# foollh/PicoPose

Measured on AMD Instinct MI355X. Metric: image-crops/sec (224x224, 162 templates), higher is better.
Workload: dtype f32 tensors; networks: f32 operands split into 2 f16 terms (22 bits) on f16 MFMA with f32 accumulate; stage-1 contraction: f16 MFMA operands, f32 accumulate, exact f32 re-evaluation of near-ties; PnP f64

## Files before the change

### include/picopose_hip.h

```cpp
#ifndef PICOPOSE_HIP_H
#define PICOPOSE_HIP_H

#include <stddef.h>
#include <stdint.h>

#ifdef __cplusplus
extern "C" {
#endif

#define PP_OK 0
#define PP_EINVAL (-1)
#define PP_EWORKSPACE (-2)
#define PP_ELAUNCH (-3)

#define PP_MATCH_EXACT 0
#define PP_MATCH_FAST 1

const char* pp_strerror(int code);
int pp_version(void);

int pp_prof_enable(int max_records);
int pp_prof_collect(float* out_ms, int max_out, int* count);
int pp_prof_gemm_enable(int max_records);
int pp_prof_gemm_collect(double* ms, double* flops, int* launches);
// ... 16 lines not shown
int pp_stage1_scores_ex(const void* bank, int bank_dtype, const float* query, const float* mask,
                        int mask_h, int mask_w, int B, int N, int C, int mode,
                        float eps, void* workspace, size_t workspace_bytes,
                        float* sim_avg, int32_t* stats, void* stream);

int pp_topk(const float* scores, int B, int N, int k, float* out_score,
            int64_t* out_index, void* stream);

int pp_stage1_match(const float* bank, const float* query, const float* mask,
                    int mask_h, int mask_w, int B, int N, int C, int k, int mode,
                    float eps, void* workspace, size_t workspace_bytes,
                    float* sim_avg, float* out_score, int64_t* out_index,
                    int32_t* stats, void* stream);
int pp_stage1_match_ex(const void* bank, int bank_dtype, const float* query, const float* mask,
                       int mask_h, int mask_w, int B, int N, int C, int k, int mode,
                       float eps, void* workspace, size_t workspace_bytes, float* sim_avg,
                       float* out_score, int64_t* out_index, int32_t* stats, void* stream);

int pp_stage1_indexed_workspace_bytes(int B, int N, int C, size_t* bytes);
int pp_stage1_scores_indexed(const void* bank, int bank_dtype, const int64_t* obj_index, int n_obj,
                             const float* query, const float* mask, int mask_h, int mask_w, int B, int N,
                             int C, int mode, float eps, void* workspace, size_t workspace_bytes,
                             float* sim_avg, int32_t* stats, void* stream);
int pp_stage1_match_indexed(const void* bank, int bank_dtype, const int64_t* obj_index, int n_obj,
                            const float* query, const float* mask, int mask_h, int mask_w, int B, int N,
                            int C, int k, int mode, float eps, void* workspace, size_t workspace_bytes,
                            float* sim_avg, float* out_score, int64_t* out_index, int32_t* stats,
                            void* stream);



int pp_similarity_volume(const float* src_feat, const float* tar_feat, const float* src_mask,
                         int mask_h, int mask_w, int B, int C, float* out, void* stream);

int pp_calc_pred_Ms(const float* pred_scale, const float* pred_inplane, const float* pred_translation,
                    const float* tem_pose, const float* tem_K, const float* tem_M, int B,
                    float trans_scale, float* pred_Ms, void* stream);

int pp_pose_recovery_2d(const float* query_M, const float* query_K, const float* pred_Ms,
                        const float* tem_K, const float* tem_M, const float* tem_pose, int B,
                        float* pred_pose, void* stream);

int pp_init_correspondences(const float* pred_Ms, const float* tem_mask, int mask_h, int mask_w, int B,
                            float* init_flow, float* init_certainty, void* stream);

int pp_stage3_correspondences(const float* pred_flow, const float* pred_certainty, int B, int H, int W,
                              float threshold, int64_t* tar_pts, int64_t* src_pts, void* stream);

int pp_gather_valid(const float* features, const int64_t* index_patches, int B, int C, int H, int W,
                    int N, float* out, int32_t* count, void* stream);

#define PP_ACT_NONE 0
#define PP_ACT_RELU 1
#define PP_ACT_GELU 2
#define PP_ACT_LEAKY01 3
#define PP_ACT_TANH 4

#define PP_PREC_F32 0
#define PP_PREC_F16X3 1
#define PP_PREC_F16 2

typedef struct PpGemmDesc {
    const float* A;
    const float* B;
    float* C;
    const float* bias;
// ... 46 lines not shown
int pp_split_weights_t(const float* w, long long n, int terms, void* out, float* scale, void* stream);
int pp_split_activation_t(const float* x, long long batch_stride, int B, int P, int row_stride, int C, int relu, void* out,
                          int ld_h, int terms, void* stream);
int pp_hl_patch_columns_t(const float* x, int ld_x, int c, long long rows, void* out, int ld_h, int col0, int terms, void* stream);
int pp_layernorm_t(const float* x, const float* gamma, const float* beta, int rows, int C, float eps, float* y, void* out, int terms,
                   void* stream);
int pp_resize_bilinear_nhwc_t(const float* in, int B, int H, int W, int C, int Ho, int Wo, float mul, void* out, int terms,
                              void* stream);
int pp_resize_bilinear_nhwc_dual(const float* in, int B, int H, int W, int C, int Ho, int Wo, float mul, float* out, void* out_operand,
                                 int terms, void* stream);
int pp_warp_nhwc_t(const float* feat, int feat_batch, const float* flow, int B, int H, int W, int C, int ld_flow, void* out,
                   int ld_h, int terms, void* stream);
int pp_attention_t(const void* qkv_operand, int terms, int B, int T, int heads, int head_dim, float scale, float* out,
                   void* out_operand, void* stream);

int pp_attention(const float* qkv, int B, int T, int heads, int head_dim, float scale, float* out, void* stream);
int pp_attention_split(const float* qkv, int B, int T, int heads, int head_dim, float scale, float* out, void* out_hl,
                       void* stream);
int pp_attention_ex(const float* qkv, int B, int T, int heads, int head_dim, float scale, int prec, float* out, void* out_hl,
                    void* stream);
int pp_attention_hl(const void* qkv_hl, int B, int T, int heads, int head_dim, float scale, float* out, void* out_hl,
                    void* stream);
int pp_attention_train(const float* qkv, int B, int T, int heads, int head_dim, float scale, float* out, float* lse2, void* stream);
int pp_attention_backward(const float* qkv, const float* out, const float* dout, const float* lse2, const float* gpair, int B, int T,
                          int heads, int head_dim, float scale, float* Dws, float* dqkv, void* stream);

int pp_layernorm(const float* x, const float* gamma, const float* beta, int rows, int C, float eps,
                 float* y, void* stream);
int pp_layernorm_split(const float* x, const float* gamma, const float* beta, int rows, int C, float eps, float* y,
                       void* hl, void* stream);
int pp_softmax_rows(float* x, int rows, int n, int ld, void* stream);
int pp_groupnorm_nhwc(const float* x, const float* gamma, const float* beta, int B, int HW, int C,
                      int groups, float eps, int relu, float* y, void* stream);
int pp_transpose_batched(const float* in, long long in_batch_stride, int B, int R, int C, float* out,
                         long long out_batch_stride, int ld_out, int col_off, void* stream);
int pp_assemble_tokens(const float* patches, const float* cls_token, const float* pos, int B, int T, int C,
                       float* tokens, void* stream);
int pp_normalize_rows(const float* x, int rows, int n, float eps, float* y, void* stream);

int pp_resize_bilinear_nhwc(const float* in, int B, int H, int W, int C, int Ho, int Wo, float mul,
                            float* out, void* stream);
int pp_resize_bilinear_nhwc_hl(const float* in, int B, int H, int W, int C, int Ho, int Wo, float mul, void* out_hl,
                               void* stream);
int pp_warp_nhwc(const float* feat, int feat_batch, const float* flow, int B, int H, int W, int C, int ld_flow,
                 float* out, int ld_out, void* stream);
int pp_warp_nhwc_hl(const float* feat, int feat_batch, const float* flow, int B, int H, int W, int C, int ld_flow,
                    void* out_hl, int ld_h, void* stream);
int pp_avgpool2_nhwc(const float* in, int B, int H, int W, int C, float* out, void* stream);
int pp_gather_rows(const float* src, const long long* index, long long n_src_rows, long long row_floats, int n, float* dst,
                   void* stream);
int pp_bank_rows_to_tokens(const float* bank, long long n_bank_rows, int C, int P, const long long* index, int n, float* tokens, int ld,
                           int T, int skip, void* stream);
int pp_patch_operand(const float* bank, long long n_bank_rows, const long long* index, int n, const float* front, int n_front, int H, int W,
                     void* out, int terms, void* stream);
int pp_flow_operand(const float* flow, int ld_flow, long long rows, void* out8, int terms, void* stream);

int pp_crop_resize_normalize(const unsigned char* image, int H, int W, const unsigned char* mask, int y1, int y2, int x1,
                             int x2, int S, int rgb_mask_flag, const double* mean3, const double* std3, float* out_rgb,
                             float* out_mask, void* stream);
int pp_depth_points_nearest(const float* depth_m, int H, int W, int y1, int y2, int x1, int x2, int P, float fx, float fy,
                            float cx, float cy, float* out_pts, void* stream);
int pp_corr_lookup_nhwc(const float* f1, int ld_f1, const float* f2_l0, const float* f2_l1, const float* f2_l2,
                        int f2_batch, const float* flow, int B, int H, int W, int C, int levels, int radius,
                        int ld_flow, float* out, int ld_out, void* stream);
int pp_corr_lookup_nhwc_ex(const float* f1, int ld_f1, const float* f2_l0, const float* f2_l1, const float* f2_l2,
                           int f2_batch, const float* flow, int B, int H, int W, int C, int levels, int radius,
// ... 322 lines not shown
```

### picopose_amd/csrc/pp_gemm.hip

```cpp

#include <hip/hip_runtime.h>
#include <stdint.h>
#include <stdio.h>
#include <stdlib.h>
#include <atomic>
#include <mutex>
#include <string>
#include <unordered_map>
#include "../../include/picopose_hip.h"
#include "pp_common.h"
#include "pp_reduce_dev.h"
#include "pp_gemm_dev.h"
#include "pp_gemm_u.h"

static std::mutex g_tune_mu;
static std::unordered_map<std::string, int> g_tune_best;
static int g_tune_loaded = 0;

static int tune_load_locked(const char* path) {
    FILE* f = fopen(path, "r");
    if (!f) return -1;
    char key[192];
    int cfg, n = 0;
    while (fscanf(f, "%191s %d", key, &cfg) == 2) {
// ... 607 lines not shown
static void launch_layernorm(const float* x, const float* gamma, const float* beta, int rows, int C, float eps, float* y,
                             _Float16* hl, hipStream_t st, int terms = 2) {
    const dim3 grid((rows + 3) / 4), block(256);
    const bool vec = C % 8 == 0 && ((uintptr_t)x % 16 == 0) && ((uintptr_t)gamma % 16 == 0) &&
                     ((uintptr_t)beta % 16 == 0) && (!y || (uintptr_t)y % 16 == 0) && (!hl || (uintptr_t)hl % 16 == 0);
    if (vec && C <= 512)
        hipLaunchKernelGGL(layernorm_kernel<1>, grid, block, 0, st, x, gamma, beta, rows, C, eps, y, hl, terms);
    else if (vec && C <= 1024)
        hipLaunchKernelGGL(layernorm_kernel<2>, grid, block, 0, st, x, gamma, beta, rows, C, eps, y, hl, terms);
    else
        hipLaunchKernelGGL(layernorm_kernel<0>, grid, block, 0, st, x, gamma, beta, rows, C, eps, y, hl, terms);
}

__global__ __launch_bounds__(256) void softmax_kernel(float* __restrict__ x, int rows, int n, int ld) {
    const int row = blockIdx.x * 4 + (threadIdx.x >> 6), lane = threadIdx.x & 63;
    if (row >= rows) return;
    float* xr = x + (size_t)row * ld;
    float mx = -INFINITY;
    for (int c = lane; c < n; c += 64) mx = fmaxf(mx, xr[c]);
    mx = wave_max(mx);
    float s = 0.f;
    for (int c = lane; c < n; c += 64) {
        const float e = expf(xr[c] - mx);
        xr[c] = e;
        s += e;
    }
    s = wave_sum(s);
    const float inv = 1.0f / s;
    for (int c = lane; c < n; c += 64) xr[c] *= inv;
}

__global__ __launch_bounds__(256) void groupnorm_kernel(const float* __restrict__ x, const float* __restrict__ g,
                                                        const float* __restrict__ b, int HW, int C, int G, float eps,
                                                        int relu, float* __restrict__ y) {
    __shared__ float red[8];
    const int img = blockIdx.x / G, grp = blockIdx.x % G, cg = C / G, tid = threadIdx.x;
    const float* xi = x + (size_t)img * HW * C + grp * cg;
    float* yi = y + (size_t)img * HW * C + grp * cg;
    const int n = HW * cg;
    float s = 0.f;
    for (int i = tid; i < n; i += 256) s += xi[(size_t)(i / cg) * C + (i % cg)];
    const float mean = block_reduce_all<4>(s, red, op_sum{}) / (float)n;
    float v = 0.f;
    for (int i = tid; i < n; i += 256) {
        const float dlt = xi[(size_t)(i / cg) * C + (i % cg)] - mean;
        v = fmaf(dlt, dlt, v);
    }
    const float rstd = 1.0f / sqrtf(block_reduce_all<4>(v, red + 4, op_sum{}) / (float)n + eps);
    for (int i = tid; i < n; i += 256) {
        const int c = i % cg;
        const size_t off = (size_t)(i / cg) * C + c;
        float o = (xi[off] - mean) * rstd * g[grp * cg + c] + b[grp * cg + c];
        if (relu) o = o > 0.f ? o : 0.f;
        yi[off] = o;
    }
}

__global__ __launch_bounds__(256) void transpose_kernel(const float* __restrict__ in, long long in_bs, int R,
                                                        int Cc, float* __restrict__ out, long long out_bs,
                                                        int ld_out, int col_off) {
    __shared__ float t[32][33];
    const int b = blockIdx.z, r0 = blockIdx.y * 32, c0 = blockIdx.x * 32;
    const int tx = threadIdx.x & 31, ty = threadIdx.x >> 5;
    const float* ib = in + (size_t)b * in_bs;
    float* ob = out + (size_t)b * out_bs;
#pragma unroll
    for (int i = 0; i < 4; ++i) {
        const int r = r0 + ty + 8 * i, c = c0 + tx;
        if (r < R && c < Cc) t[ty + 8 * i][tx] = ib[(size_t)r * Cc + c];
    }
    __syncthreads();
#pragma unroll
    for (int i = 0; i < 4; ++i) {
        const int c = c0 + ty + 8 * i, r = r0 + tx;
        if (r < R && c < Cc) ob[(size_t)c * ld_out + col_off + r] = t[tx][ty + 8 * i];
    }
}

__global__ __launch_bounds__(256) void assemble_tokens_kernel(const float* __restrict__ patches,
                                                              const float* __restrict__ cls,
                                                              const float* __restrict__ pos, int T, int C,
                                                              float* __restrict__ tokens) {
    const int t = blockIdx.x, b = blockIdx.y;
    const float* src = t == 0 ? cls : patches + ((size_t)b * T + (t - 1)) * C;
    float* dst = tokens + ((size_t)b * (T + 1) + t) * C;
    for (int c = threadIdx.x; c < C; c += 256) dst[c] = src[c] + pos[(size_t)t * C + c];
}
// ... 638 lines not shown
    return (int)g_tune_best.size();
}

int pp_layernorm(const float* x, const float* gamma, const float* beta, int rows, int C, float eps, float* y,
                 void* stream) {
    if (!x || !gamma || !beta || !y || rows <= 0 || C <= 0) return PP_EINVAL;
    launch_layernorm(x, gamma, beta, rows, C, eps, y, nullptr, (hipStream_t)stream);
    return pp_last_launch();
}

int pp_layernorm_t(const float* x, const float* gamma, const float* beta, int rows, int C, float eps, float* y,
                   void* hl, int terms, void* stream) {
    if (!x || !gamma || !beta || !hl || rows <= 0 || C <= 0 || C % 8 != 0 || (terms != 1 && terms != 2)) return PP_EINVAL;
    launch_layernorm(x, gamma, beta, rows, C, eps, y, (_Float16*)hl, (hipStream_t)stream, terms);
    return pp_last_launch();
}

int pp_layernorm_split(const float* x, const float* gamma, const float* beta, int rows, int C, float eps, float* y,
                       void* hl, void* stream) {
    return pp_layernorm_t(x, gamma, beta, rows, C, eps, y, hl, 2, stream);
}

int pp_softmax_rows(float* x, int rows, int n, int ld, void* stream) {
    if (!x || rows <= 0 || n <= 0 || ld < n) return PP_EINVAL;
    hipLaunchKernelGGL(softmax_kernel, dim3((rows + 3) / 4), dim3(256), 0, (hipStream_t)stream, x, rows, n, ld);
    return pp_last_launch();
}

int pp_groupnorm_nhwc(const float* x, const float* gamma, const float* beta, int B, int HW, int C, int groups,
                      float eps, int relu, float* y, void* stream) {
    if (!x || !gamma || !beta || !y || B <= 0 || HW <= 0 || C <= 0 || groups <= 0 || C % groups != 0)
        return PP_EINVAL;
    hipLaunchKernelGGL(groupnorm_kernel, dim3(B * groups), dim3(256), 0, (hipStream_t)stream, x, gamma, beta, HW,
                       C, groups, eps, relu, y);
    return pp_last_launch();
}

int pp_transpose_batched(const float* in, long long in_batch_stride, int B, int R, int C, float* out,
                         long long out_batch_stride, int ld_out, int col_off, void* stream) {
    if (!in || !out || B <= 0 || R <= 0 || C <= 0 || ld_out < R + col_off || col_off < 0) return PP_EINVAL;
    if (in_batch_stride == 0) in_batch_stride = (long long)R * C;
    if (out_batch_stride == 0) out_batch_stride = (long long)C * ld_out;
    hipLaunchKernelGGL(transpose_kernel, dim3((C + 31) / 32, (R + 31) / 32, B), dim3(256), 0,
                       (hipStream_t)stream, in, in_batch_stride, R, C, out, out_batch_stride, ld_out, col_off);
    return pp_last_launch();
}

int pp_assemble_tokens(const float* patches, const float* cls_token, const float* pos, int B, int T, int C,
                       float* tokens, void* stream) {
    if (!patches || !cls_token || !pos || !tokens || B <= 0 || T <= 0 || C <= 0) return PP_EINVAL;
    hipLaunchKernelGGL(assemble_tokens_kernel, dim3(T + 1, B), dim3(256), 0, (hipStream_t)stream, patches,
                       cls_token, pos, T, C, tokens);
    return pp_last_launch();
}

int pp_normalize_rows(const float* x, int rows, int n, float eps, float* y, void* stream) {
    if (!x || !y || rows <= 0 || n <= 0 || n > 64) return PP_EINVAL;
    hipLaunchKernelGGL(normalize_rows_kernel, dim3((rows + 255) / 256), dim3(256), 0, (hipStream_t)stream, x,
                       rows, n, eps, y);
    return pp_last_launch();
}

}
```

### picopose_amd/csrc/pp_geom.hip

```cpp

#include <hip/hip_runtime.h>
#include <stdint.h>
#include "../../include/picopose_hip.h"
#include "pp_common.h"

namespace {

typedef float f32x16 __attribute__((ext_vector_type(16)));
typedef float f4 __attribute__((ext_vector_type(4)));

__device__ __forceinline__ int nearest16(int dst, int in) {
    int i = (int)floorf((float)dst * ((float)in / 16.0f));
    return i < in - 1 ? i : in - 1;
}

__global__ __launch_bounds__(256) void simvol_kernel(const float* __restrict__ src,
                                                     const float* __restrict__ tar,
                                                     const float* __restrict__ src_mask, int mh,
                                                     int mw, int C, float* __restrict__ out) {
    __shared__ __attribute__((aligned(16))) float Qs[16 * 128];
    __shared__ __attribute__((aligned(16))) float Xs[16 * 128];
    __shared__ float rq[128], rx[128];
    const int b = blockIdx.x, t0 = blockIdx.y * 128, s0 = blockIdx.z * 128;
    const int tid = threadIdx.x, lane = tid & 63, w = tid >> 6;
    const int wr = w >> 1, wc = w & 1, l31 = lane & 31, lh = lane >> 5;
    const float* qg = tar + (size_t)b * C * 256 + t0;
    const float* xg = src + (size_t)b * C * 256 + s0;
    f32x16 acc[2][2];
#pragma unroll
    for (int i = 0; i < 2; ++i)
#pragma unroll
        for (int j = 0; j < 2; ++j)
#pragma unroll
            for (int r = 0; r < 16; ++r) acc[i][j][r] = 0.f;
    float sa[2] = {0.f, 0.f}, sb[2] = {0.f, 0.f};
    for (int c0 = 0; c0 < C; c0 += 16) {
#pragma unroll
        for (int j = 0; j < 2; ++j) {
            const int idx = tid + 256 * j, row = idx >> 5, col = (idx & 31) * 4;
            *(f4*)(Qs + row * 128 + col) = *(const f4*)(qg + (size_t)(c0 + row) * 256 + col);
            *(f4*)(Xs + row * 128 + col) = *(const f4*)(xg + (size_t)(c0 + row) * 256 + col);
        }
        __syncthreads();
#pragma unroll
        for (int p = 0; p < 8; ++p) {
            float a[2], bv[2];
#pragma unroll
            for (int i = 0; i < 2; ++i) {
                a[i] = Qs[(2 * p + lh) * 128 + wr * 64 + i * 32 + l31];
                bv[i] = Xs[(2 * p + lh) * 128 + wc * 64 + i * 32 + l31];
                sa[i] = fmaf(a[i], a[i], sa[i]);
                sb[i] = fmaf(bv[i], bv[i], sb[i]);
            }
#pragma unroll
            for (int i = 0; i < 2; ++i)
#pragma unroll
                for (int j = 0; j < 2; ++j)
                    acc[i][j] = __builtin_amdgcn_mfma_f32_32x32x2f32(a[i], bv[j], acc[i][j], 0, 0, 0);
        }
        __syncthreads();
    }
#pragma unroll
    for (int i = 0; i < 2; ++i) {
        sa[i] += __shfl_xor(sa[i], 32);
        sb[i] += __shfl_xor(sb[i], 32);
    }
    if (lh == 0) {
        if (wc == 0) {
            rq[wr * 64 + l31] = 1.0f / fmaxf(sqrtf(sa[0]), 1e-12f);
            rq[wr * 64 + 32 + l31] = 1.0f / fmaxf(sqrtf(sa[1]), 1e-12f);
        }
        if (wr == 0) {
#pragma unroll
            for (int i = 0; i < 2; ++i) {
                const int s = s0 + wc * 64 + i * 32 + l31;
                const float m = src_mask[((size_t)b * mh + nearest16(s >> 4, mh)) * mw + nearest16(s & 15, mw)];
                rx[wc * 64 + i * 32 + l31] = m / fmaxf(sqrtf(sb[i]), 1e-12f);
            }
        }
    }
    __syncthreads();
#pragma unroll
    for (int j = 0; j < 2; ++j) {
        const int sl = wc * 64 + j * 32 + l31;
        const float cs = rx[sl];
        float* o = out + ((size_t)b * 256 + s0 + sl) * 256;
#pragma unroll
        for (int i = 0; i < 2; ++i)
#pragma unroll
            for (int e = 0; e < 16; ++e) {
                const int tl = wr * 64 + i * 32 + (e & 3) + 8 * (e >> 2) + 4 * lh;
                const int t = t0 + tl;
                float v = acc[i][j][e] * rq[tl] * cs;
                v = v < 0.f ? 0.f : v;
                o[(t & 15) * 16 + (t >> 4)] = v;
            }
    }
}

struct M3 {
    float m[9];
};
__device__ __forceinline__ M3 ld3(const float* p) {
    M3 r;
#pragma unroll
    for (int i = 0; i < 9; ++i) r.m[i] = p[i];
    return r;
}
__device__ __forceinline__ M3 mul3(const M3& a, const M3& b) {
    M3 r;
#pragma unroll
    for (int i = 0; i < 3; ++i)
#pragma unroll
        for (int j = 0; j < 3; ++j)
            r.m[i * 3 + j] = a.m[i * 3] * b.m[j] + a.m[i * 3 + 1] * b.m[3 + j] + a.m[i * 3 + 2] * b.m[6 + j];
    return r;
}
__device__ __forceinline__ void mulv3(const M3& a, const float* v, float* o) {
#pragma unroll
    for (int i = 0; i < 3; ++i) o[i] = a.m[i * 3] * v[0] + a.m[i * 3 + 1] * v[1] + a.m[i * 3 + 2] * v[2];
}

__global__ void pred_ms_kernel(const float* __restrict__ scale, const float* __restrict__ inplane,
                               const float* __restrict__ trans, const float* __restrict__ tem_pose,
                               const float* __restrict__ tem_K, const float* __restrict__ tem_M, int B,
                               float trans_scale, float* __restrict__ out) {
    const int b = blockIdx.x * blockDim.x + threadIdx.x;
    if (b >= B) return;
    const float* P = tem_pose + (size_t)b * 16;
    const float t[3] = {P[3], P[7], P[11]};
// ... 117 lines not shown
            y = ib[2 * n + 1];
        }
        const bool v = x != -1 && y != -1;
        const unsigned long long bal = __ballot(v);
        const int pre = __popcll(bal & ((1ull << lane) - 1ull));
        if (lane == 0) wsum[wv] = __popcll(bal);
        __syncthreads();
        int off = base;
        for (int i = 0; i < wv; ++i) off += wsum[i];
        if (v) {
            const int r = off + pre;
            const int64_t p = y * W + x;
            for (int c = 0; c < C; ++c) ob[(size_t)r * C + c] = fb[(size_t)c * H * W + p];
        }
        __syncthreads();
        if (tid == 0) {
            int t = base;
            for (int i = 0; i < 16; ++i) t += wsum[i];
            base = t;
        }
        __syncthreads();
    }
    if (tid == 0) count[b] = base;
}

}

extern "C" {

int pp_similarity_volume(const float* src_feat, const float* tar_feat, const float* src_mask, int mask_h,
                         int mask_w, int B, int C, float* out, void* stream) {
    if (!src_feat || !tar_feat || !src_mask || !out) return PP_EINVAL;
    if (B <= 0 || C <= 0 || C % 16 != 0 || mask_h <= 0 || mask_w <= 0) return PP_EINVAL;
    hipLaunchKernelGGL(simvol_kernel, dim3(B, 2, 2), dim3(256), 0, (hipStream_t)stream, src_feat, tar_feat,
                       src_mask, mask_h, mask_w, C, out);
    return pp_last_launch();
}

int pp_calc_pred_Ms(const float* pred_scale, const float* pred_inplane, const float* pred_translation,
                    const float* tem_pose, const float* tem_K, const float* tem_M, int B, float trans_scale,
                    float* pred_Ms, void* stream) {
    if (!pred_scale || !pred_inplane || !pred_translation || !tem_pose || !tem_K || !tem_M || !pred_Ms || B <= 0)
        return PP_EINVAL;
    hipLaunchKernelGGL(pred_ms_kernel, dim3((B + 63) / 64), dim3(64), 0, (hipStream_t)stream, pred_scale,
                       pred_inplane, pred_translation, tem_pose, tem_K, tem_M, B, trans_scale, pred_Ms);
    return pp_last_launch();
}

int pp_pose_recovery_2d(const float* query_M, const float* query_K, const float* pred_Ms, const float* tem_K,
                        const float* tem_M, const float* tem_pose, int B, float* pred_pose, void* stream) {
    if (!query_M || !query_K || !pred_Ms || !tem_K || !tem_M || !tem_pose || !pred_pose || B <= 0)
        return PP_EINVAL;
    hipLaunchKernelGGL(pose2d_kernel, dim3((B + 63) / 64), dim3(64), 0, (hipStream_t)stream, query_M, query_K,
                       pred_Ms, tem_K, tem_M, tem_pose, B, pred_pose);
    return pp_last_launch();
}

int pp_init_correspondences(const float* pred_Ms, const float* tem_mask, int mask_h, int mask_w, int B,
                            float* init_flow, float* init_certainty, void* stream) {
    if (!pred_Ms || !tem_mask || !init_flow || !init_certainty || B <= 0) return PP_EINVAL;
    if (mask_h != mask_w || mask_h < 16) return PP_EINVAL;
    hipLaunchKernelGGL(init_corr_kernel, dim3(B), dim3(256), 0, (hipStream_t)stream, pred_Ms, tem_mask,
                       mask_h, mask_w, init_flow, init_certainty);
    return pp_last_launch();
}

int pp_stage3_correspondences(const float* pred_flow, const float* pred_certainty, int B, int H, int W,
                              float threshold, int64_t* tar_pts, int64_t* src_pts, void* stream) {
// ... 17 lines not shown
```

### picopose_amd/model/stage2.py

```python
import torch

from .. import ops
from .common import Packed, conv_p, linear_p, norm_p, seq


def _head(hidden, out):
    return seq((0, linear_p(hidden, hidden)), (2, linear_p(hidden, hidden)), (4, linear_p(hidden, out)))


class AffineRegressor(Packed):
    def __init__(self, cfg, use_tanh_act=True, normalize_output=True):
        super().__init__()
        self.in_channel, self.hidden_dim = cfg.in_channel, cfg.hidden_dim
        self.feat_size = 8
        hd = self.hidden_dim
        self.features = seq((0, conv_p(self.in_channel, hd, 1)), (1, norm_p(hd)), (3, conv_p(hd, hd, 3, bias=False)),
                            (4, norm_p(hd)))
        self.fc1 = linear_p(hd * self.feat_size * self.feat_size, 1024)
        self.fc2 = linear_p(1024, 256)
        self.translation_predictor = _head(hd, 2)
        self.scale_predictor = _head(hd, 1)
        self.inplane_predictor = _head(hd, 2)

    def _pack(self):
        f = self.features
        hd, fs = self.hidden_dim, self.feat_size
        fc1 = self.fc1.weight.float().view(-1, hd, fs, fs).permute(0, 2, 3, 1).reshape(-1, fs * fs * hd).contiguous()
        return {"c0": ops.pack_conv_weight(getattr(f, "0").weight.float()),
                "c3": ops.pack_conv_weight(getattr(f, "3").weight.float()), "fc1": fc1}

    def _mlp(self, head, x, last_act=None):
        l0, l2, l4 = getattr(head, "0"), getattr(head, "2"), getattr(head, "4")
        x = ops.linear(x, l0.weight, l0.bias, act="relu")
        x = ops.linear(x, l2.weight, l2.bias, act="relu")
        return ops.linear(x, l4.weight, l4.bias, act=last_act)

    def forward(self, x):
        with torch.no_grad():
            pk, f = self.packed(), self.features
            B = x.shape[0]
            h = ops.conv2d(ops.to_nhwc(x), pk["c0"], getattr(f, "0").bias, 1)
            h = ops.groupnorm(h, getattr(f, "1").weight, getattr(f, "1").bias, 32, relu=True)
            h = ops.conv2d(h, pk["c3"], None, 3, stride=2, pad=1)
            h = ops.groupnorm(h, getattr(f, "4").weight, getattr(f, "4").bias, 32, relu=True)
            h = ops.linear_splitk(h.view(B, -1), pk["fc1"], self.fc1.bias, act="leaky01")
            h = ops.linear(h, self.fc2.weight, self.fc2.bias, act="leaky01")
            translation = self._mlp(self.translation_predictor, h)
            scale = self._mlp(self.scale_predictor, h)
            inplane = ops.normalize_rows(self._mlp(self.inplane_predictor, h, last_act="tanh"))
            return translation, scale.squeeze(1), inplane
```

### picopose_amd/ops.py

```python
import contextlib
import ctypes
import os
import threading

import torch

from . import _lib
from ._lib import PpGemmDesc

ACT = {None: 0, "none": 0, "relu": 1, "gelu": 2, "leaky01": 3, "tanh": 4}

PRECISION = "f16x3"
_PREC = {"f32": 0, "f16x3": 1, "f16": 2}
_split_cache = {}
_scope = threading.local()


def precision():
    return getattr(_scope, "mode", None) or PRECISION


def check_precision(mode):
    if mode is not None and mode not in _PREC:
        raise ValueError(f"unknown arithmetic mode {mode!r}: expected None or one of {sorted(_PREC)}")
# ... 892 lines not shown
        out = torch.empty(B * T, heads * hd, dtype=torch.float32, device=dev)
    if isinstance(qkv, Split):
        _lib.call("pp_attention_t", qkv.hl, qkv.terms, B, T, heads, hd, float(hd) ** -0.5, out, sp.hl if sp else None)
    else:
        assert qkv.is_contiguous()
        if sp is not None and sp.terms == 1:
            sp, out = None, torch.empty(B * T, heads * hd, dtype=torch.float32, device=dev)
        _lib.call("pp_attention_ex", qkv, B, T, heads, hd, float(hd) ** -0.5, _fly_prec(), out, sp.hl if sp else None)
    if sp is not None:
        _chk(sp.hl, "pp_attention")
    return sp if sp is not None else out


def layernorm(x, weight, bias, eps, out_split=False):
    rows, C = x.shape
    assert x.is_contiguous()
    if out_split and _split_ok(C):
        sp = Split.empty(rows, C, x.device)
        _lib.call("pp_layernorm_t", x, weight, bias, rows, C, float(eps), None, sp.hl, sp.terms)
        _chk(sp.hl, "pp_layernorm_t")
        return sp
    y = torch.empty_like(x)
    _lib.call("pp_layernorm", x, weight, bias, rows, C, float(eps), y)
    return y


def softmax_rows_(x):
    assert x.is_contiguous()
    n = x.shape[-1]
    _lib.call("pp_softmax_rows", x, x.numel() // n, n, n)
    return x


def groupnorm(x, weight, bias, groups, eps=1e-5, relu=False):
    B, H, W, C = x.shape
    assert x.is_contiguous()
    y = torch.empty_like(x)
    _lib.call("pp_groupnorm_nhwc", x, weight, bias, B, H * W, C, groups, float(eps), int(relu), y)
    return y


def batchnorm_train(x, bn, relu=False, residual=None, residual2=None, eps=1e-5, momentum=0.1):
    assert x.is_contiguous() and x.dtype == torch.float32
    C = x.shape[-1]
    rows = x.numel() // C
    nbytes = _lib.lib().pp_batchnorm_train_workspace_bytes(rows, C)
    ws = torch.empty(nbytes, dtype=torch.uint8, device=x.device)
    y = torch.empty_like(x)
    for r in (residual, residual2):
        assert r is None or (r.is_contiguous() and r.shape == x.shape)
    _lib.call("pp_batchnorm_train", x, bn.weight, bn.bias, rows, C, float(eps), float(momentum), bn.running_mean, bn.running_var,
              int(relu), residual, residual2, y, ws, nbytes)
    bn.num_batches_tracked += 1
    return y


def to_nhwc(x, c_pad=None):
    B, C, H, W = x.shape
    x = x.contiguous().float()
    Cp = c_pad if c_pad and c_pad > C else C
    out = (torch.zeros if Cp > C else torch.empty)(B, H, W, Cp, dtype=torch.float32, device=x.device)
    _lib.call("pp_transpose_batched", x, 0, B, C, H * W, out, 0, Cp, 0)
    return out


def to_nchw(x):
    B, H, W, C = x.shape
    assert x.is_contiguous()
    out = torch.empty(B, C, H, W, dtype=torch.float32, device=x.device)
# ... 37 lines not shown
            _chk(tgt.cols(col0, C), "pp_warp_nhwc_t")
        return None
    if out is None:
        out = torch.empty(B, H, W, C, dtype=torch.float32, device=feat.device)
    _lib.call("pp_warp_nhwc", feat, Bf, flow, B, H, W, C, flow.stride(2), out, out.stride(2))
    return out


def avgpool2(x):
    B, H, W, C = x.shape
    assert x.is_contiguous()
    out = torch.empty(B, H // 2, W // 2, C, dtype=torch.float32, device=x.device)
    _lib.call("pp_avgpool2_nhwc", x, B, H, W, C, out)
    return out


def avgpool2_hl(x, keep_f32=True):
    B, H, W, C = x.shape
    assert x.is_contiguous() and C % 8 == 0 and terms() == 2
    out = torch.empty(B, H // 2, W // 2, C, dtype=torch.float32, device=x.device) if keep_f32 else None
    sp = Split.empty(B * (H // 2) * (W // 2), C, x.device)
    sp.image = (B, H // 2, W // 2)
    _lib.call("pp_avgpool2_hl", x, B, H, W, C, out, sp.hl)
    _chk(sp.hl, "pp_avgpool2_hl")
    return out, sp


def corr_operand_out():
    return os.environ.get("PP_CORR_OPERAND_OUT", "1") != "0"


def decoder_lean():
    return os.environ.get("PP_DECODER_LEAN", "1") != "0"


def corr_takes_operands(f1_hl, f2_hl, H, W, C):
    return (f1_hl is not None and f2_hl is not None and precision() == "f16x3" and f2_hl.terms == 2 and H % 8 == 0 and W % 8 == 0 and C % 32 == 0
            and os.environ.get("PP_CORR_TILED", "1") != "0" and os.environ.get("PP_CORR_HL", "1") != "0")


def _corr_pyramid(f2, hl0, levels, fused):
    C = f2.shape[3]
    pyr, hls = [f2], [hl0]
    for i in range(levels - 1):
        if fused:
            p, sp = avgpool2_hl(pyr[-1], keep_f32=i < levels - 2)
            hls.append(sp.hl)
        else:
            p = avgpool2(pyr[-1])
            if hl0 is not None:
                hls.append(split_activation(p, p.shape[0], p.shape[1] * p.shape[2], C, p.shape[1] * p.shape[2] * C, C))
        pyr.append(p)
    return pyr + [None, None], hls + [None, None]


def corr_lookup(f1, f2, flow, levels, radius, c_pad=None, f1_hl=None, f2_hl=None, out_split=False):
    (H, W, C), B = f2.shape[1:], flow.shape[0]
    assert f2.is_contiguous() and flow.stride(3) == 1 and B % f2.shape[0] == 0 and tuple(flow.shape[1:3]) == (H, W)
    operands = corr_takes_operands(f1_hl, f2_hl, H, W, C)
    if f1 is None:
        assert operands, "corr_lookup without the fp32 map f1 needs the operand form of both maps (corr_takes_operands)"
    else:
        assert tuple(f1.shape) == (B, H, W, C) and f1.stride(3) == 1 and f1.stride(1) == W * f1.stride(2) and f1.stride(0) == H * f1.stride(1)
    n = levels * (2 * radius + 1) ** 2
    np_ = c_pad if c_pad and c_pad > n else n
    assert not out_split or (operands and np_ % 8 == 0), "corr_lookup(out_split=True) needs the operand branch and a padded channel count"
# ... 77 lines not shown
```

### picopose_amd/picopose.py

```python
import os

import torch
import torch.nn as nn

from . import ops
from .model.stage1 import FeatureExtractor
from .model.stage2 import AffineRegressor
from .model.stage3 import OffsetRegressor
from .utils.augment import aug_gtM_noise
from .utils.correspondence import compute_init_correspondences, compute_stage3_correspondences
from .utils.keypoints import KeypointInput, KeyPointSampler
from .utils.loss_utils import compute_stage_two_loss, flow_level_losses, infonce_rows
from .utils.matching import matching_features_similarity, matching_templates, matching_templates_indexed
from .utils.pose_recovery import pose_recovery_2d_prediction
from .utils.torch_utils import calc_pred_Ms


BATCH_VIT_TRAIN = os.environ.get("PP_BATCH_VIT_TRAIN", "1") != "0"
BATCH_DPT = os.environ.get("PP_BATCH_DPT", "1") != "0"
PREFETCH_QUERY = os.environ.get("PP_PREFETCH_QUERY", "1") != "0"
TEMPLATE_LAST_FROM_BANK = {"0": False, "1": True}.get(os.environ.get("PP_TEMPLATE_LAST_FROM_BANK"))


def _tensor_key(t, fe=None):
    key = (t.data_ptr(), tuple(t.shape), t._version, ops.precision())
    return key if fe is None else key + (fe._signatures()[0],)


def _image_rows(p, b0, b1):
    if isinstance(p, ops.Split):
        hw = p.image[1] * p.image[2]
        s = ops.Split(p.hl[b0 * hw:b1 * hw], p.terms)
        s.image = (b1 - b0,) + tuple(p.image[1:])
        return s
    q = p[b0:b1]
    hl = getattr(p, "_hl", None)
    if hl is not None:
        hw = p.shape[1] * p.shape[2]
        s = ops.Split(hl.hl[b0 * hw:b1 * hw], hl.terms)
        s.image = (b1 - b0, p.shape[1], p.shape[2])
        q._hl = s
    return q


class Net(nn.Module):
    def __init__(self, cfg):
# ... 69 lines not shown
        real_dpt = real[2] if len(real) > 2 else None
        levels = real[3] if len(real) > 3 else None
        output = {"tem_pose": end_points["tem_pose"]}
        output["tar_pts_2d"] = end_points["real_pts2d"].permute(0, 3, 2, 1)
        output["src_pts_3d"] = end_points["tem_pts3d"].permute(0, 3, 1, 2)
        pre = real[4] if len(real) > 4 else None
        bank = end_points.get("tem_bank") if tem_cached is None else None
        T = h0 * w0 + 1
        rgb_rows = end_points.get("tem_rgb_rows")

        def tem_images(front=None):
            if rgb_rows is not None and ops.patch_operand_ok(rgb_rows[0], front):
                return ops.patch_operand(*rgb_rows, front=front)
            tem = end_points["tem_rgb"] if rgb_rows is None else ops.gather_rows(*rgb_rows)
            return tem if front is None else torch.cat([front, tem])

        if tem_cached is None and pre is not None and levels is not None:
            alloc, nxt = pre
            Bn = nxt.shape[0]
            both, _ = fe.forward_tokens(tem_images(nxt), level_out=(alloc, 0), full_depth=None if bank is None else Bn)
            tem_tok = [t[Bn:] for t in both]
            if bank is not None:
                nT = tem_tok[0].shape[0]
                tem_tok[-1] = ops.bank_rows_to_tokens(*bank, T, out=alloc[-1][Bn * T:(Bn + nT) * T]).view(nT, T, -1)
            self._query_stash = (_tensor_key(nxt, fe), [a[:Bn * T].clone() for a in alloc], (h0, w0), nxt)
        elif tem_cached is None:
            tem_tok, _ = fe.forward_tokens(tem_images(), level_out=None if levels is None else (levels, 0),
                                           full_depth=None if bank is None else 0)
            if bank is not None:
                nT = tem_tok[0].shape[0]
                tem_tok[-1] = ops.bank_rows_to_tokens(*bank, T, out=None if levels is None else levels[-1][:nT * T]).view(nT, T, -1)
        else:
            tem_last, tem_dpt = tem_cached
        if tem_cached is None:
            tem_last = ops.tokens_to_nchw(tem_tok[-1], 1, h0, w0) if bank is None else ops.gather_rows(*bank)
        sim = matching_features_similarity(tem_last, ops.tokens_to_nchw(real_tok[-1], 1, h0, w0),
                                           end_points["tem_mask"], end_points["real_mask"])
        pred_translation, pred_scale, pred_inplane = self.affine_regressor(sim)
        pred_Ms = calc_pred_Ms(pred_scale, pred_inplane, pred_translation, end_points["tem_pose"], end_points["tem_K"],
                               end_points["tem_M"])
        output["pred_poses"] = pose_recovery_2d_prediction(end_points["real_M"], end_points["real_K"], pred_Ms,
                                                           end_points["tem_K"], end_points["tem_M"], end_points["tem_pose"])
        init_flow, init_certainty = compute_init_correspondences(pred_Ms, end_points["tem_mask"])
        as_img = lambda t: t[:, 1:].unflatten(1, (h0, w0))
        orr = self.offset_regressor
        if levels is not None and real_dpt is None and tem_cached is None:
            nT, nR = tem_tok[0].shape[0], levels[0].shape[0] // T - tem_tok[0].shape[0]
            both = orr.dpt_head.forward_nhwc([as_img(lv.view(-1, T, lv.shape[1])) for lv in levels], finest_operand_only=True)
            tem_dpt, real_dpt = [_image_rows(p_, 0, nT) for p_ in both], [_image_rows(p_, nT, nT + nR) for p_ in both]
        else:
            if real_dpt is None:
                real_dpt = orr.dpt_head.forward_nhwc([as_img(t) for t in real_tok])
            if tem_cached is None:
                tem_dpt = orr.dpt_head.forward_nhwc([as_img(t) for t in tem_tok])
        flows, certs = orr.flow_decoder.forward_nhwc(tem_dpt, real_dpt, ops.to_nhwc(init_flow), ops.to_nhwc(init_certainty))
        if self.keep_stage3:
            self.last_stage3 = (flows[-1], certs[-1])
        output["pred_tar_pts"], output["pred_src_pts"] = compute_stage3_correspondences(
            ops.to_nchw(flows[-1]), ops.to_nchw(certs[-1]), threshold=0.5)
        return output

    def forward_hypotheses(self, end_points, pred_id_src, real):
        hyp = pred_id_src.shape[1]
        cache = end_points.get("template_cache")
        tidx = end_points.get("template_index")

        def cached(rows, idx):
            if cache is None:
                return None
            obj = (cache["obj_index"] if tidx is None else tidx)[rows]
            return end_points["template_feature"][rows if tidx is None else obj, idx], [m[obj, idx] for m in cache["dpt"]]

        if not self.batch_hypotheses:
            rows = torch.arange(pred_id_src.shape[0], device=pred_id_src.device)
            return [self.forward_test_hyp(self.select_template_data(end_points, pred_id_src, k), real,
                                          cached(rows, pred_id_src[:, k])) for k in range(hyp)]
        real_tok, hw = real[0], real[1]
        real_dpt = real[2] if len(real) > 2 and real[2] is not None else None
        levels = real[3] if len(real) > 3 else None
        B = pred_id_src.shape[0]
        idx = pred_id_src.t().reshape(-1)
        rows = torch.arange(B, device=idx.device).repeat(hyp)
        rep = lambda t: t.repeat(hyp, *([1] * (t.dim() - 1)))
        N = end_points["tem_pose"].shape[1]
        trow = rows if tidx is None else tidx[rows]
        flat = trow * N + idx
        rgb_rows = None
        if (ops.patch_operand_on() and not self.training and cache is None and levels is not None and end_points["tem_rgb"].dim() == 5
                and end_points["tem_rgb"].is_contiguous() and flat.dtype == torch.int64 and ops.patch_operand_ok(end_points["tem_rgb"].flatten(0, 1))):
            rgb_rows = (end_points["tem_rgb"].flatten(0, 1), flat)
        sel = {key: (ops.gather_rows(end_points[key].flatten(0, 1), flat) if end_points[key].is_contiguous()
                     else end_points[key][trow, idx])
               for key in ("tem_pose", "tem_K", "tem_M", "tem_mask", "tem_rgb", "tem_pts3d") if not (key == "tem_rgb" and rgb_rows is not None)}
        if rgb_rows is not None:
            sel["tem_rgb_rows"] = rgb_rows
        if self._last_from_bank(end_points):
            sel["tem_bank"] = (end_points["template_feature"].flatten(0, 1), flat)
        for key in ("real_pts2d", "real_K", "real_M", "real_mask", "real_pose"):
            sel[key] = rep(end_points[key])
        toks = ([rep(t) for t in real_tok] if real_dpt is None and levels is None
                else [None] * (len(real_tok) - 1) + [rep(real_tok[-1])])
        out = self.forward_test_hyp(sel, (toks, hw, real_dpt, levels if cache is None else None, real[4] if len(real) > 4 and cache is None else None),
                                    cached(rows, idx))
        return [{key: v[k * B:(k + 1) * B] for key, v in out.items()} for k in range(hyp)]

    TEMPLATE_KEYS = ("template_feature", "tem_pose", "tem_K", "tem_M", "tem_mask", "tem_rgb", "tem_pts3d")

    def _check_template_index(self, end_points):
        tidx = end_points["template_index"]
        B = end_points["real_rgb"].shape[0]
        if not isinstance(tidx, torch.Tensor) or tidx.dtype != torch.int64 or tuple(tidx.shape) != (B,) or tidx.device != end_points["real_rgb"].device:
            raise ValueError(f"template_index must be a ({B},) int64 tensor on the crops' device")
        lead = {key: tuple(end_points[key].shape[:2]) for key in self.TEMPLATE_KEYS if key in end_points}
        if len(set(lead.values())) != 1:
            raise ValueError(f"with template_index every template tensor is (O, N, ...) for the same O and N: {lead}")
        cache = end_points.get("template_cache")
        if cache is not None and cache["obj_index"] is not tidx and not torch.equal(cache["obj_index"].to(tidx.device), tidx):
            raise ValueError("template_cache['obj_index'] and template_index name different objects")

    def forward_test(self, end_points, hyp=5, next_real_rgb=None):
        with torch.no_grad():
            if "template_index" in end_points:
                self._check_template_index(end_points)
            fe = self.feature_extractor
            levels = None
            ops.saturation_word(end_points["real_rgb"].device)
            stash, self._query_stash = getattr(self, "_query_stash", None), None
            if BATCH_DPT and self.batch_hypotheses and end_points.get("template_cache") is None:
                B, _, H, W = end_points["real_rgb"].shape
                T = (H // fe.patch_size) * (W // fe.patch_size) + 1
                pre_ok = PREFETCH_QUERY and next_real_rgb is not None and tuple(next_real_rgb.shape[1:]) == (3, H, W) and next_real_rgb.is_contiguous()
                Bn = next_real_rgb.shape[0] if pre_ok else 0
                alloc = [torch.empty((Bn + (hyp + 1) * B) * T, fe.num_features, dtype=torch.float32, device=end_points["real_rgb"].device)
                         for _ in fe.blocks_to_take]
# ... 97 lines not shown
```

### picopose_amd/utils/matching.py

```python
import torch

from .. import _lib

DEFAULT_MODE = "fast"
_MODES = {"exact": _lib.PP_MATCH_EXACT, "fast": _lib.PP_MATCH_FAST}

_ws_cache = {}


def _workspace(B, N, C, device, query="pp_stage1_workspace_bytes"):
    need = _lib.workspace_bytes(query, B, N, C)
    key = (device.index, torch.cuda.current_stream().cuda_stream)
    ws = _ws_cache.get(key)
    if ws is None or ws.numel() < need:
        ws = torch.empty(need, dtype=torch.uint8, device=device)
        _ws_cache[key] = ws
    return ws, need


def _check_inputs(src_feats, tar_feat, tar_mask):
    if not (src_feats.is_cuda and tar_feat.is_cuda and tar_mask.is_cuda):
        raise _lib.PicoPoseHipError("picopose_amd runs on the GPU only: inputs must be CUDA(HIP) tensors")
    B, N, C, H, W = src_feats.shape
    assert H == W
# ... 101 lines not shown
class MatchingGraph:

    def __init__(self, src_feats, tar_feat, tar_mask, topk=5, mode=None):
        _check_inputs(src_feats, tar_feat, tar_mask)
        for t in (src_feats, tar_feat, tar_mask):
            if not t.is_contiguous():
                raise _lib.PicoPoseHipError("MatchingGraph reads its inputs in place: they must be contiguous")
        if src_feats.dtype not in (torch.float16, torch.float32) or tar_feat.dtype != torch.float32 or tar_mask.dtype != torch.float32:
            raise _lib.PicoPoseHipError("MatchingGraph reads its inputs in place: fp32 query / mask, fp32 or fp16 bank")
        self.inputs = (src_feats, tar_feat, tar_mask)
        self.graph = torch.cuda.CUDAGraph()
        side = torch.cuda.Stream()
        side.wait_stream(torch.cuda.current_stream())
        with torch.cuda.stream(side):
            matching_templates(src_feats, tar_feat, None, tar_mask, topk=topk, mode=mode)
        torch.cuda.current_stream().wait_stream(side)
        with torch.cuda.graph(self.graph):
            self.score, self.index = matching_templates(src_feats, tar_feat, None, tar_mask, topk=topk, mode=mode)

    def __call__(self):
        self.graph.replay()
        return self.score, self.index


def matching_features_similarity(src_feat, tar_feat, src_mask, tar_mask):
    B, C, H, W = src_feat.shape
    assert H == W
    if H != 16:
        raise _lib.PicoPoseHipError("the HIP similarity-volume kernel is built for 16x16 patch grids")
    src, tar, mask = _lib.dev_f32(src_feat, tar_feat, src_mask)
    out = torch.empty(B, H * W, H, W, dtype=torch.float32, device=src.device)
    _lib.call("pp_similarity_volume", src, tar, mask, mask.shape[1], mask.shape[2], B, C, out)
    return out
```

Baseline: 593.4.

## Emit stage-2 similarity volume and groupnorm outputs directly as split f16 operands

The similarity-volume kernel gains an operand mode. It reads query tokens and bank rows in place through an index and writes split f16 GEMM operands directly, which removes the gather_rows, tokens_to_nchw, repeat and later split conversions. The kernel also prefetches the next channel tile into registers so loads overlap compute. Groupnorm and the fc2/MLP first layers emit split outputs as well, which avoids separate conversion passes. The cost is more code paths plus a transposed shared-memory store for the query tile, and the new paths depend on the env flags and presplit mode.

Result: no change. 597.1, median of 6 (+0.6%).

```diff
diff --git a/include/picopose_hip.h b/include/picopose_hip.h
--- a/include/picopose_hip.h
+++ b/include/picopose_hip.h
@@ -72,6 +72,9 @@
 
 int pp_similarity_volume(const float* src_feat, const float* tar_feat, const float* src_mask,
                          int mask_h, int mask_w, int B, int C, float* out, void* stream);
+int pp_similarity_volume_operand(const float* bank, long long n_bank_rows, const long long* index, const float* query_tokens,
+                                 long long query_image_stride, int query_ld, int Bq, const float* src_mask, int mask_h, int mask_w, int B,
+                                 int C, void* out, int terms, void* stream);
 
 int pp_calc_pred_Ms(const float* pred_scale, const float* pred_inplane, const float* pred_translation,
                     const float* tem_pose, const float* tem_K, const float* tem_M, int B,
@@ -184,6 +187,8 @@
 int pp_softmax_rows(float* x, int rows, int n, int ld, void* stream);
 int pp_groupnorm_nhwc(const float* x, const float* gamma, const float* beta, int B, int HW, int C,
                       int groups, float eps, int relu, float* y, void* stream);
+int pp_groupnorm_nhwc_t(const float* x, const float* gamma, const float* beta, int B, int HW, int C, int groups, float eps, int relu,
+                        float* y, void* hl, int terms, void* stream);
 int pp_transpose_batched(const float* in, long long in_batch_stride, int B, int R, int C, float* out,
                          long long out_batch_stride, int ld_out, int col_off, void* stream);
 int pp_assemble_tokens(const float* patches, const float* cls_token, const float* pos, int B, int T, int C,
diff --git a/picopose_amd/csrc/pp_gemm.hip b/picopose_amd/csrc/pp_gemm.hip
--- a/picopose_amd/csrc/pp_gemm.hip
+++ b/picopose_amd/csrc/pp_gemm.hip
@@ -663,7 +663,7 @@
 
 __global__ __launch_bounds__(256) void groupnorm_kernel(const float* __restrict__ x, const float* __restrict__ g,
                                                         const float* __restrict__ b, int HW, int C, int G, float eps,
-                                                        int relu, float* __restrict__ y) {
+                                                        int relu, float* __restrict__ y, _Float16* __restrict__ hl, int terms) {
     __shared__ float red[8];
     const int img = blockIdx.x / G, grp = blockIdx.x % G, cg = C / G, tid = threadIdx.x;
     const float* xi = x + (size_t)img * HW * C + grp * cg;
@@ -683,7 +683,19 @@
         const size_t off = (size_t)(i / cg) * C + c;
         float o = (xi[off] - mean) * rstd * g[grp * cg + c] + b[grp * cg + c];
         if (relu) o = o > 0.f ? o : 0.f;
-        yi[off] = o;
+        if (y) yi[off] = o;
+        if (hl) {
+            _Float16 h, l;
+            pp_split_f16_chk(o, h, l);
+            const size_t row = (size_t)img * HW + i / cg;
+            if (terms == 2) {
+                _Float16* hp = hl + row * 2 * C + pp_hl_col(grp * cg + c, 0);
+                hp[0] = h;
+                hp[8] = l;
+            } else {
+                hl[row * C + grp * cg + c] = h;
+            }
+        }
     }
 }
 
@@ -1388,7 +1400,17 @@
     if (!x || !gamma || !beta || !y || B <= 0 || HW <= 0 || C <= 0 || groups <= 0 || C % groups != 0)
         return PP_EINVAL;
     hipLaunchKernelGGL(groupnorm_kernel, dim3(B * groups), dim3(256), 0, (hipStream_t)stream, x, gamma, beta, HW,
-                       C, groups, eps, relu, y);
+                       C, groups, eps, relu, y, nullptr, 0);
+    return pp_last_launch();
+}
+
+int pp_groupnorm_nhwc_t(const float* x, const float* gamma, const float* beta, int B, int HW, int C, int groups, float eps, int relu,
+                        float* y, void* hl, int terms, void* stream) {
+    if (!x || !gamma || !beta || !hl || B <= 0 || HW <= 0 || C <= 0 || groups <= 0 || C % groups != 0 || C % 8 != 0 ||
+        ((uintptr_t)hl % 16) != 0 || (terms != 1 && terms != 2))
+        return PP_EINVAL;
+    hipLaunchKernelGGL(groupnorm_kernel, dim3(B * groups), dim3(256), 0, (hipStream_t)stream, x, gamma, beta, HW,
+                       C, groups, eps, relu, y, (_Float16*)hl, terms);
     return pp_last_launch();
 }
 
diff --git a/picopose_amd/csrc/pp_geom.hip b/picopose_amd/csrc/pp_geom.hip
--- a/picopose_amd/csrc/pp_geom.hip
+++ b/picopose_amd/csrc/pp_geom.hip
@@ -14,18 +14,25 @@
     return i < in - 1 ? i : in - 1;
 }
 
-__global__ __launch_bounds__(256) void simvol_kernel(const float* __restrict__ src,
-                                                     const float* __restrict__ tar,
-                                                     const float* __restrict__ src_mask, int mh,
-                                                     int mw, int C, float* __restrict__ out) {
-    __shared__ __attribute__((aligned(16))) float Qs[16 * 128];
+template <bool OPERAND>
+__global__ __launch_bounds__(256) void simvol_kernel(const float* __restrict__ src, const long long* __restrict__ index, long long n_rows,
+                                                     const float* __restrict__ tar, long long q_bs, int q_ld, int Bq,
+                                                     const float* __restrict__ src_mask, int mh, int mw, int C, void* __restrict__ out_,
+                                                     int terms) {
+    constexpr int QLD = OPERAND ? 132 : 128;
+    __shared__ __attribute__((aligned(16))) float Qs[16 * QLD];
     __shared__ __attribute__((aligned(16))) float Xs[16 * 128];
     __shared__ float rq[128], rx[128];
     const int b = blockIdx.x, t0 = blockIdx.y * 128, s0 = blockIdx.z * 128;
     const int tid = threadIdx.x, lane = tid & 63, w = tid >> 6;
     const int wr = w >> 1, wc = w & 1, l31 = lane & 31, lh = lane >> 5;
-    const float* qg = tar + (size_t)b * C * 256 + t0;
-    const float* xg = src + (size_t)b * C * 256 + s0;
+    long long xrow = b;
+    if constexpr (OPERAND) {
+        if (index) xrow = index[b];
+        if (xrow < 0 || xrow >= n_rows) return;
+    }
+    const float* qg = OPERAND ? tar + (size_t)(b % Bq) * q_bs + (size_t)t0 * q_ld : tar + (size_t)b * C * 256 + t0;
+    const float* xg = src + (size_t)xrow * C * 256 + s0;
     f32x16 acc[2][2];
 #pragma unroll
     for (int i = 0; i < 2; ++i)
@@ -34,20 +41,37 @@
 #pragma unroll
             for (int r = 0; r < 16; ++r) acc[i][j][r] = 0.f;
     float sa[2] = {0.f, 0.f}, sb[2] = {0.f, 0.f};
+    f4 qn[2], xn[2];
+#define PP_SIMVOL_FETCH(C0)                                                                                          \
+    _Pragma("unroll") for (int j = 0; j < 2; ++j) {                                                                  \
+        const int idx = tid + 256 * j, row = idx >> 5, col = (idx & 31) * 4;                                         \
+                                      \
+        qn[j] = OPERAND ? *(const f4*)(qg + (size_t)(idx >> 2) * q_ld + (C0) + (idx & 3) * 4)                        \
+                        : *(const f4*)(qg + (size_t)((C0) + row) * 256 + col);                                       \
+        xn[j] = *(const f4*)(xg + (size_t)((C0) + row) * 256 + col);                                                 \
+    }
+    PP_SIMVOL_FETCH(0)
     for (int c0 = 0; c0 < C; c0 += 16) {
 #pragma unroll
         for (int j = 0; j < 2; ++j) {
             const int idx = tid + 256 * j, row = idx >> 5, col = (idx & 31) * 4;
-            *(f4*)(Qs + row * 128 + col) = *(const f4*)(qg + (size_t)(c0 + row) * 256 + col);
-            *(f4*)(Xs + row * 128 + col) = *(const f4*)(xg + (size_t)(c0 + row) * 256 + col);
-        }
-        __syncthreads();
+            if constexpr (OPERAND) {
+                const int tk = idx >> 2, cq = (idx & 3) * 4;
+#pragma unroll
+                for (int k = 0; k < 4; ++k) Qs[(cq + k) * QLD + tk] = qn[j][k];
+            } else {
+                *(f4*)(Qs + row * QLD + col) = qn[j];
+            }
+            *(f4*)(Xs + row * 128 + col) = xn[j];
+        }
+        __syncthreads();
+        if (c0 + 16 < C) PP_SIMVOL_FETCH(c0 + 16)
 #pragma unroll
         for (int p = 0; p < 8; ++p) {
             float a[2], bv[2];
 #pragma unroll
             for (int i = 0; i < 2; ++i) {
-                a[i] = Qs[(2 * p + lh) * 128 + wr * 64 + i * 32 + l31];
+                a[i] = Qs[(2 * p + lh) * QLD + wr * 64 + i * 32 + l31];
                 bv[i] = Xs[(2 * p + lh) * 128 + wc * 64 + i * 32 + l31];
                 sa[i] = fmaf(a[i], a[i], sa[i]);
                 sb[i] = fmaf(bv[i], bv[i], sb[i]);
@@ -60,6 +84,7 @@
         }
         __syncthreads();
     }
+#undef PP_SIMVOL_FETCH
 #pragma unroll
     for (int i = 0; i < 2; ++i) {
         sa[i] += __shfl_xor(sa[i], 32);
@@ -80,11 +105,13 @@
         }
     }
     __syncthreads();
+    bool bad = false;
 #pragma unroll
     for (int j = 0; j < 2; ++j) {
         const int sl = wc * 64 + j * 32 + l31;
         const float cs = rx[sl];
-        float* o = out + ((size_t)b * 256 + s0 + sl) * 256;
+        float* o = (float*)out_ + ((size_t)b * 256 + s0 + sl) * 256;
+        _Float16* oh = (_Float16*)out_ + (size_t)b * 256 * 256 * terms + (terms == 2 ? pp_hl_col(s0 + sl, 0) : s0 + sl);
 #pragma unroll
         for (int i = 0; i < 2; ++i)
 #pragma unroll
@@ -93,9 +120,20 @@
                 const int t = t0 + tl;
                 float v = acc[i][j][e] * rq[tl] * cs;
                 v = v < 0.f ? 0.f : v;
-                o[(t & 15) * 16 + (t >> 4)] = v;
+                if constexpr (OPERAND) {
+                    _Float16* p = oh + (size_t)((t & 15) * 16 + (t >> 4)) * 256 * terms;
+                    bad |= !(fabsf(v) * PP_A_SCALE < 65504.f);
+                    if (terms == 2) {
+                        pp_split_f16(v, p[0], p[8]);
+                    } else {
+                        p[0] = pp_to_f16(v);
+                    }
+                } else {
+                    o[(t & 15) * 16 + (t >> 4)] = v;
+                }
             }
     }
+    if constexpr (OPERAND) pp_sat_flag(bad);
 }
 
 struct M3 {
@@ -279,8 +317,21 @@
                          int mask_w, int B, int C, float* out, void* stream) {
     if (!src_feat || !tar_feat || !src_mask || !out) return PP_EINVAL;
     if (B <= 0 || C <= 0 || C % 16 != 0 || mask_h <= 0 || mask_w <= 0) return PP_EINVAL;
-    hipLaunchKernelGGL(simvol_kernel, dim3(B, 2, 2), dim3(256), 0, (hipStream_t)stream, src_feat, tar_feat,
-                       src_mask, mask_h, mask_w, C, out);
+    hipLaunchKernelGGL(simvol_kernel<false>, dim3(B, 2, 2), dim3(256), 0, (hipStream_t)stream, src_feat, nullptr, 0, tar_feat, 0, 0, 1,
+                       src_mask, mask_h, mask_w, C, out, 0);
+    return pp_last_launch();
+}
+
+int pp_similarity_volume_operand(const float* bank, long long n_bank_rows, const long long* index, const float* query_tokens,
+                                 long long query_image_stride, int query_ld, int Bq, const float* src_mask, int mask_h, int mask_w, int B,
+                                 int C, void* out, int terms, void* stream) {
+    if (!bank || !query_tokens || !src_mask || !out) return PP_EINVAL;
+    if (B <= 0 || Bq <= 0 || C <= 0 || C % 16 != 0 || mask_h <= 0 || mask_w <= 0 || (terms != 1 && terms != 2)) return PP_EINVAL;
+    if (n_bank_rows <= 0 || (!index && n_bank_rows < B)) return PP_EINVAL;
+    if (query_ld < C || query_ld % 4 != 0 || query_image_stride % 4 != 0 || query_image_stride < 0) return PP_EINVAL;
+    if (((uintptr_t)bank | (uintptr_t)query_tokens | (uintptr_t)out) % 16 != 0) return PP_EINVAL;
+    hipLaunchKernelGGL(simvol_kernel<true>, dim3(B, 2, 2), dim3(256), 0, (hipStream_t)stream, bank, index, n_bank_rows, query_tokens,
+                       query_image_stride, query_ld, Bq, src_mask, mask_h, mask_w, C, out, terms);
     return pp_last_launch();
 }
 
diff --git a/picopose_amd/model/stage2.py b/picopose_amd/model/stage2.py
--- a/picopose_amd/model/stage2.py
+++ b/picopose_amd/model/stage2.py
@@ -29,23 +29,24 @@
         return {"c0": ops.pack_conv_weight(getattr(f, "0").weight.float()),
                 "c3": ops.pack_conv_weight(getattr(f, "3").weight.float()), "fc1": fc1}
 
-    def _mlp(self, head, x, last_act=None):
+    def _mlp(self, head, x, last_act=None, lean=False):
         l0, l2, l4 = getattr(head, "0"), getattr(head, "2"), getattr(head, "4")
-        x = ops.linear(x, l0.weight, l0.bias, act="relu")
+        x = ops.linear(x, l0.weight, l0.bias, act="relu", out_split=lean)
         x = ops.linear(x, l2.weight, l2.bias, act="relu")
         return ops.linear(x, l4.weight, l4.bias, act=last_act)
 
     def forward(self, x):
         with torch.no_grad():
             pk, f = self.packed(), self.features
-            B = x.shape[0]
-            h = ops.conv2d(ops.to_nhwc(x), pk["c0"], getattr(f, "0").bias, 1)
-            h = ops.groupnorm(h, getattr(f, "1").weight, getattr(f, "1").bias, 32, relu=True)
+            lean = ops.stage2_lean() and ops.presplit()
+            B = x.image[0] if isinstance(x, ops.Split) else x.shape[0]
+            h = ops.conv2d(x if isinstance(x, ops.Split) else ops.to_nhwc(x), pk["c0"], getattr(f, "0").bias, 1)
+            h = ops.groupnorm(h, getattr(f, "1").weight, getattr(f, "1").bias, 32, relu=True, out_split=lean)
             h = ops.conv2d(h, pk["c3"], None, 3, stride=2, pad=1)
             h = ops.groupnorm(h, getattr(f, "4").weight, getattr(f, "4").bias, 32, relu=True)
             h = ops.linear_splitk(h.view(B, -1), pk["fc1"], self.fc1.bias, act="leaky01")
-            h = ops.linear(h, self.fc2.weight, self.fc2.bias, act="leaky01")
-            translation = self._mlp(self.translation_predictor, h)
-            scale = self._mlp(self.scale_predictor, h)
-            inplane = ops.normalize_rows(self._mlp(self.inplane_predictor, h, last_act="tanh"))
+            h = ops.linear(h, self.fc2.weight, self.fc2.bias, act="leaky01", out_split=lean)
+            translation = self._mlp(self.translation_predictor, h, lean=lean)
+            scale = self._mlp(self.scale_predictor, h, lean=lean)
+            inplane = ops.normalize_rows(self._mlp(self.inplane_predictor, h, last_act="tanh", lean=lean))
             return translation, scale.squeeze(1), inplane
diff --git a/picopose_amd/ops.py b/picopose_amd/ops.py
--- a/picopose_amd/ops.py
+++ b/picopose_amd/ops.py
@@ -948,9 +948,15 @@
     return x
 
 
-def groupnorm(x, weight, bias, groups, eps=1e-5, relu=False):
+def groupnorm(x, weight, bias, groups, eps=1e-5, relu=False, out_split=False):
     B, H, W, C = x.shape
     assert x.is_contiguous()
+    if out_split and _split_ok(C):
+        sp = Split.empty(B * H * W, C, x.device)
+        sp.image = (B, H, W)
+        _lib.call("pp_groupnorm_nhwc_t", x, weight, bias, B, H * W, C, groups, float(eps), int(relu), None, sp.hl, sp.terms)
+        _chk(sp.hl, "pp_groupnorm_nhwc_t")
+        return sp
     y = torch.empty_like(x)
     _lib.call("pp_groupnorm_nhwc", x, weight, bias, B, H * W, C, groups, float(eps), int(relu), y)
     return y
@@ -1054,6 +1060,10 @@
 
 def decoder_lean():
     return os.environ.get("PP_DECODER_LEAN", "1") != "0"
+
+
+def stage2_lean():
+    return os.environ.get("PP_STAGE2_LEAN", "1") != "0"
 
 
 def corr_takes_operands(f1_hl, f2_hl, H, W, C):
diff --git a/picopose_amd/picopose.py b/picopose_amd/picopose.py
--- a/picopose_amd/picopose.py
+++ b/picopose_amd/picopose.py
@@ -11,7 +11,8 @@
 from .utils.correspondence import compute_init_correspondences, compute_stage3_correspondences
 from .utils.keypoints import KeypointInput, KeyPointSampler
 from .utils.loss_utils import compute_stage_two_loss, flow_level_losses, infonce_rows
-from .utils.matching import matching_features_similarity, matching_templates, matching_templates_indexed
+from .utils.matching import (matching_features_similarity, matching_templates, matching_templates_indexed, similarity_volume_operand,
+                             similarity_volume_operand_ok)
 from .utils.pose_recovery import pose_recovery_2d_prediction
 from .utils.torch_utils import calc_pred_Ms
 
@@ -147,10 +148,19 @@
                 tem_tok[-1] = ops.bank_rows_to_tokens(*bank, T, out=None if levels is None else levels[-1][:nT * T]).view(nT, T, -1)
         else:
             tem_last, tem_dpt = tem_cached
-        if tem_cached is None:
-            tem_last = ops.tokens_to_nchw(tem_tok[-1], 1, h0, w0) if bank is None else ops.gather_rows(*bank)
-        sim = matching_features_similarity(tem_last, ops.tokens_to_nchw(real_tok[-1], 1, h0, w0),
-                                           end_points["tem_mask"], end_points["real_mask"])
+        if tem_cached is None and bank is None:
+            tem_last = ops.tokens_to_nchw(tem_tok[-1], 1, h0, w0)
+        src = bank if bank is not None else (tem_last, None)
+        if ops.stage2_lean() and similarity_volume_operand_ok(real_tok[-1], *src):
+            sim = similarity_volume_operand(real_tok[-1], src[0], end_points["tem_mask"], src[1])
+        else:
+            if bank is not None:
+                tem_last = ops.gather_rows(*bank)
+            real_last = real_tok[-1]
+            if real_last.shape[0] != tem_last.shape[0]:
+                real_last = real_last.repeat(tem_last.shape[0] // real_last.shape[0], 1, 1)
+            sim = matching_features_similarity(tem_last, ops.tokens_to_nchw(real_last, 1, h0, w0),
+                                               end_points["tem_mask"], end_points["real_mask"])
         pred_translation, pred_scale, pred_inplane = self.affine_regressor(sim)
         pred_Ms = calc_pred_Ms(pred_scale, pred_inplane, pred_translation, end_points["tem_pose"], end_points["tem_K"],
                                end_points["tem_M"])
@@ -214,7 +224,7 @@
         for key in ("real_pts2d", "real_K", "real_M", "real_mask", "real_pose"):
             sel[key] = rep(end_points[key])
         toks = ([rep(t) for t in real_tok] if real_dpt is None and levels is None
-                else [None] * (len(real_tok) - 1) + [rep(real_tok[-1])])
+                else [None] * (len(real_tok) - 1) + [real_tok[-1] if ops.stage2_lean() and ops.presplit() else rep(real_tok[-1])])
         out = self.forward_test_hyp(sel, (toks, hw, real_dpt, levels if cache is None else None, real[4] if len(real) > 4 and cache is None else None),
                                     cached(rows, idx))
         return [{key: v[k * B:(k + 1) * B] for key, v in out.items()} for k in range(hyp)]
diff --git a/picopose_amd/utils/matching.py b/picopose_amd/utils/matching.py
--- a/picopose_amd/utils/matching.py
+++ b/picopose_amd/utils/matching.py
@@ -157,3 +157,28 @@
     out = torch.empty(B, H * W, H, W, dtype=torch.float32, device=src.device)
     _lib.call("pp_similarity_volume", src, tar, mask, mask.shape[1], mask.shape[2], B, C, out)
     return out
+
+
+def similarity_volume_operand_ok(query_tokens, src, index=None, skip=1):
+    from .. import ops
+
+    ok = lambda t: t.dtype == torch.float32 and t.is_contiguous() and t.is_cuda and t.data_ptr() % 16 == 0
+    return (ops.presplit() and query_tokens.dim() == 3 and ok(query_tokens) and query_tokens.shape[1] >= skip + 256
+            and src.dim() == 4 and ok(src) and tuple(src.shape[1:]) == (query_tokens.shape[2], 16, 16) and src.shape[1] % 16 == 0
+            and (index is None or (index.dtype == torch.int64 and index.dim() == 1 and index.device == src.device)))
+
+
+def similarity_volume_operand(query_tokens, src, src_mask, index=None, skip=1):
+    from .. import ops
+
+    assert similarity_volume_operand_ok(query_tokens, src, index, skip)
+    Bq, T, C = query_tokens.shape
+    B = src.shape[0] if index is None else index.numel()
+    mask = _lib.dev_f32(src_mask)[0]
+    assert mask.dim() == 3 and mask.shape[0] == B
+    sp = ops.Split.empty(B * 256, 256, src.device)
+    sp.image = (B, 16, 16)
+    _lib.call("pp_similarity_volume_operand", src, src.shape[0], None if index is None else index.contiguous(), query_tokens[:, skip:],
+              T * C, C, Bq, mask, mask.shape[1], mask.shape[2], B, C, sp.hl, sp.terms)
+    ops._chk(sp.hl, "pp_similarity_volume_operand")
+    return sp
```
